# ViennaRNA/RNAcode

Measured on AMD Instinct MI355X. Metric: alignment-columns x samples scored /sec, higher is better.
Workload: dtype f32; 1 GPU; synthetic MAF 10000 blocks x 120 cols x 6 seqs, n=1000 (BASELINE configs[2]/[3]); exchange=none, fit_exp_mode=fused

## Files before the change

rnacode_amd/csrc/rc_null_kernel.h:

```cpp
#pragma once
#include <hip/hip_runtime.h>

#include <type_traits>
#include <utility>

#include "rc_device.h"
#include "rc_launch.h"

namespace rc {


template <bool SEM> __device__ __forceinline__ float ref_max(float x, float y) {
  if constexpr (SEM) return x > y ? x : y;
  else return fmaxf(x, y);
}
template <bool SEM> __device__ __forceinline__ float ref_max3(float x, float y, float z) { return ref_max<SEM>(ref_max<SEM>(x, y), z); }

template <bool SEM = false>
__device__ __forceinline__ void pair_step(int zc, float sig, float Delta, float Omega, float omega,
                                          float &s0, float &s1, float &s2) {
  if (zc == 0) {
    s0 = s0 + sig;
    s1 = s1 + omega;
    s2 = s2 + omega;
  } else if (zc == 1) {
    const float n0 = ref_max<SEM>(s0 + Delta, s2 + Omega);
    const float n1 = ref_max<SEM>(s0 + Omega, s1 + Delta);
    const float n2 = ref_max<SEM>(s1 + Omega, s2 + Delta);
    s0 = n0; s1 = n1; s2 = n2;
  } else {
    const float n0 = ref_max<SEM>(s0 + Delta, s1 + Omega);
    const float n1 = ref_max<SEM>(s1 + Delta, s2 + Omega);
    const float n2 = ref_max<SEM>(s2 + Delta, s0 + Omega);
    s0 = n0; s1 = n1; s2 = n2;
  }
}

struct ScanState {
  float cm;
  int ss, se;
};

template <typename Emit>
__device__ __forceinline__ void scan_step(ScanState &st, float v, int a, int j, bool last, float tieThr, Emit emit) {
  if (v > 0.0f || last) {
    if ((st.cm > 0.0f && st.se < a) || last) {
      if (st.se - st.ss >= 2) emit(st);
      st.cm = v; st.ss = a; st.se = j;
    } else if (v > st.cm || (fabsf(v - st.cm) < tieThr && (j - a) >= (st.se - st.ss))) {
      st.cm = v; st.ss = a; st.se = j;
    }
  }
}

__device__ __forceinline__ void native_scan_rows(const float *rows, int aLo, int aHi, int sites, int s, int f, float tieThr, ScanState &st, int &n,
                                                 DevHss *out, int hssCap, int lane) {
  for (int a = aLo; a < aHi; a++) {
    for (int j0 = a; j0 < sites; j0 += kWave) {
      const int j = j0 + lane;
      const float v = (j < sites) ? rows[static_cast<size_t>(a - aLo) * sites + j] : 0.0f;
      const bool last = (a == sites - 1) && (j == sites - 1);
      unsigned long long m = __ballot((j < sites) && (v > 0.0f || last));
      while (m) {
        const int t = __builtin_ctzll(m);
        m &= m - 1ull;
        const int jj = j0 + t;
        const float vt = __int_as_float(__builtin_amdgcn_readlane(__float_as_int(v), t));
        scan_step(st, vt, a, jj, (a == sites - 1) && (jj == sites - 1), tieThr, [&](const ScanState &e) {
          if (out && lane == 0 && n < hssCap) out[n] = DevHss{s, f, e.ss, e.se, e.cm};
          n++;
        });
      }
    }
  }
}

__device__ __forceinline__ uint32_t codon_flip(uint32_t c) { return ((c & 3u) << 4) | (c & 12u) | ((c >> 4) & 3u); }


template <int K> struct KReg { float s0, s1, s2; int lut; };
template <typename Seq> struct KRegs;
template <int... K> struct KRegs<std::integer_sequence<int, K...>> : KReg<K>... {
  template <int I> __device__ __forceinline__ KReg<I> &at() { return static_cast<KReg<I> &>(*this); }
};
template <int NK, typename F, int... K>
__device__ __forceinline__ void static_for_impl(F &&f, std::integer_sequence<int, K...>) {
  (f(std::integral_constant<int, K>{}), ...);
}
template <int NK, typename F> __device__ __forceinline__ void static_for(F &&f) {
  static_for_impl<NK>(static_cast<F &&>(f), std::make_integer_sequence<int, NK>{});
}

template <int NK, bool EXACT> __device__ __forceinline__ float div_by_nk(float x, float nkf) {
  if constexpr ((NK & (NK - 1)) == 0) {
    return x * (1.0f / static_cast<float>(NK));
  } else if constexpr (EXACT) {
    return x / nkf;
  } else {
    constexpr float y = 1.0f / static_cast<float>(NK);
    const float q0 = x * y;
    const float r = __builtin_fmaf(-static_cast<float>(NK), q0, x);
    return __builtin_fmaf(r, y, q0);
  }
}

struct SampleScan {
  float cm;
  float Q;
  uint32_t se;
  uint32_t len;
};
__device__ __forceinline__ void sample_scan_row_begin(SampleScan &st, float &best, uint32_t a) {
  const bool done = (st.cm > 0.0f) & (st.se < a);
  best = (done & (st.len >= 2u) & (st.cm > best)) ? st.cm : best;
  st.cm = done ? 0.0f : st.cm;
  st.len = done ? 0u : st.len;
  st.Q = static_cast<float>(2u * (st.len + a));
}
__device__ __forceinline__ void sample_scan_step(SampleScan &st, float v, float j2, float negTieThr) {
  const float d = v - st.cm;
  const bool upd = (v > st.cm) | ((v > 0.0f) & (d > negTieThr) & (st.Q <= j2));
  st.cm = upd ? v : st.cm;
  st.Q = upd ? j2 : st.Q;
}
__device__ __forceinline__ void sample_scan_row_end(SampleScan &st, uint32_t a) {
  const uint32_t q = static_cast<uint32_t>(st.Q);
  const bool inrow = (q & 1u) != 0u;
  const uint32_t j = q >> 1;
  st.se = inrow ? j : st.se;
  st.len = inrow ? j - a : st.len;
}
__device__ __forceinline__ void sample_scan_last(const SampleScan &st, float &best) {
  best = ((st.len >= 2u) & (st.cm > best)) ? st.cm : best;
}

struct DeepFetch {};
template <int OFF> struct StagedSite { uint32_t at; };
template <typename T> struct IsStagedSite : std::false_type {};
template <int OFF> struct IsStagedSite<StagedSite<OFF>> : std::true_type {};
template <int OFF> constexpr int staged_off(StagedSite<OFF>) { return OFF; }
__device__ __forceinline__ int site_index(int j) { return j; }
template <int OFF> __device__ __forceinline__ int site_index(StagedSite<OFF>) { return 0; }

template <int NK, bool LDSC, bool EXACT, bool DUAL, int MODE = 0>
__device__ __forceinline__ void null_body(const NullArgs &A, const uint8_t *__restrict__ blob,
                                          const DevBlock *__restrict__ dblocks, const int *__restrict__ classBlocks,
                                          const uint32_t *__restrict__ flags, const uint32_t *__restrict__ Ustream, const uint8_t *__restrict__ pairTab,
                                          uint32_t *__restrict__ scratch, float *__restrict__ maxima) {
  constexpr int N = NK + 1;
  constexpr int CPW = 5;
  constexpr int NCW = (NK + CPW - 1) / CPW;
  constexpr bool kTableLookups = !LDSC && !EXACT;
  constexpr int kTableWords = kTableLookups ? NK * kWave : 0;
  constexpr int LB = code_tail_bytes(NK);
  constexpr int PSW = code_pos_words(NK);
  using TailT = std::conditional_t<LB == 1, uint8_t, std::conditional_t<LB == 2, uint16_t, uint32_t>>;
  constexpr int ZW = (NK + 31) / 32;
  using Regs = KRegs<std::make_integer_sequence<int, NK>>;
  static_assert(!DUAL || (!EXACT && NK <= kDualRowsMaxNK), "two rows per pass: fast division, few sequences");
  static_assert(!(LDSC && EXACT), "the EXACT instantiation uses no LDS");
  constexpr bool ROWS = MODE == 1, SIM = MODE == 2;
#ifndef RC_DEEP_FETCH_MAX_NK
#define RC_DEEP_FETCH_MAX_NK 31
#endif
  constexpr bool kDeep = !LDSC && !EXACT && !DUAL && MODE == 0 && NK <= RC_DEEP_FETCH_MAX_NK;
  static_assert(MODE == 0 || (!LDSC && !EXACT && !DUAL), "rows split over workgroups: the one-row kernel that reads its codes from L2");
  extern __shared__ uint32_t lds_codes[];

  const int lane = threadIdx.x;
  unsigned int xcc;
  asm volatile("s_getreg_b32 %0, hwreg(HW_REG_XCC_ID)" : "=s"(xcc));
  const int home = static_cast<int>(xcc & 7u);
  const int rowParts = ROWS ? A.rowParts : 1;
  const int parts = SIM ? A.simParts : A.comboSplit ? 6 * rowParts : 1;
  const int nBlocks = A.nBlocksPtr ? *A.nBlocksPtr : A.nClassBlocks;
  const bool stealing = A.steal != nullptr && !A.comboSplit;
  constexpr int kStealHdr = 16;
  auto claim_part = [&](int slot) -> int {
    unsigned int v = 0;
    if (lane == 0) v = atomicAdd(A.steal + kStealHdr + slot, 1u);
    v = static_cast<unsigned int>(__builtin_amdgcn_readfirstlane(static_cast<int>(v)));
    return (v >= 1u && v <= 6u) ? static_cast<int>(v) - 1 : 6;
  };
  auto steal_word = [&](size_t at) -> unsigned int { return __hip_atomic_load(A.steal + at, __ATOMIC_RELAXED, __HIP_MEMORY_SCOPE_AGENT); };
  int helpCursor = 0;
  bool helping = false;
  for (int qi = 0;;) {
    int bi, grp, onlyCombo = -1, firstCombo = 0, rowPart = 0, itemIndex = 0;
    bool shared = false;
    int slot = static_cast<int>(blockIdx.x);
    if (!helping) {
      if (qi >= 8) {
        if (!stealing) break;
        helping = true;
        continue;
      }
      const int q = (home + qi) & 7;
      const int g0 = A.gLo + ((q - A.gLo) & 7);
      const int gq = g0 < A.gHi ? ((A.gHi - 1 - g0) >> 3) + 1 : 0;
      const int perBlock = gq * parts;
      const int nq = nBlocks * perBlock;
      int t = nq;
      if (nq > 0) {
        if (lane == 0) t = static_cast<int>(atomicAdd((SIM ? A.simCounter : A.workCounter) + q, 1u));
        t = __builtin_amdgcn_readfirstlane(t);
      }
      if (t >= nq) { qi++; continue; }
      bi = classBlocks[t / perBlock];
      if (A.skipMask && (flags[bi] & A.skipMask)) continue;
      const int sub = t % perBlock;
      grp = g0 + 8 * (sub / parts);
      onlyCombo = A.comboSplit ? (sub % parts) / rowParts : -1;
      if constexpr (MODE != 0) { rowPart = SIM ? sub % parts : (sub % parts) % rowParts; itemIndex = (t / perBlock) * (A.gHi - A.gLo) + (grp - A.gLo); }
      if constexpr (MODE != 0) slot = itemIndex;
      if (stealing && nq - t <= static_cast<int>(gridDim.x >> 3) + 16) {
        shared = true;
        if (lane == 0) atomicAdd(A.steal + 1, 1u);
      }
    } else {
      const size_t G = gridDim.x;
      const int np = __builtin_amdgcn_readfirstlane(static_cast<int>(steal_word(0)));
      int victim = -1;
      while (helpCursor < np) {
        const int i = helpCursor + lane;
        const unsigned int ent = i < np ? steal_word(kStealHdr + 3 * G + i) : 0u;
        const bool foreign = ent != 0u && (ent >> 24) != static_cast<unsigned int>(home);
        const unsigned int e = ent & 0xFFFFFFu;
        const unsigned int v = (e && !foreign) ? steal_word(kStealHdr + e - 1) : 0u;
        const unsigned long long open = __ballot(v >= 1u && v <= 6u);
        if (open) {
          int pick = static_cast<int>(blockIdx.x % static_cast<unsigned int>(__builtin_popcountll(open)));
          unsigned long long m = open;
          while (pick--) m &= m - 1ull;
          victim = __builtin_amdgcn_readlane(static_cast<int>(e), __builtin_ctzll(m)) - 1;
          break;
        }
        const unsigned long long notDone = ~__ballot(e != 0u && (v > 6u || foreign));
        const int adv = notDone ? __builtin_ctzll(notDone) : kWave;
        helpCursor += adv;
        if (adv < kWave) break;
      }
      if (victim < 0) {
        if (!A.stealWait) break;
        if (helpCursor >= np && steal_word(1) == 0u && static_cast<int>(steal_word(0)) == np) break;
        __builtin_amdgcn_s_sleep(127);
        continue;
      }
      firstCombo = claim_part(victim);
      if (firstCombo >= 6) continue;
      __atomic_thread_fence(__ATOMIC_ACQUIRE);
      shared = true;
      slot = victim;
      bi = __builtin_amdgcn_readfirstlane(static_cast<int>(steal_word(kStealHdr + G + 2 * victim)));
      grp = __builtin_amdgcn_readfirstlane(static_cast<int>(steal_word(kStealHdr + G + 2 * victim + 1)));
    }
    uint32_t *__restrict__ cod = scratch + static_cast<size_t>(slot) * A.scratchStride;
    const DevBlock *__restrict__ db = dblocks + bi;
    const bool nanSem = EXACT && (flags[bi] & kFlagNan) != 0u;
    const int cols = db->cols, L = db->L, nnodes = db->nnodes;
    const float Delta = db->Delta, Omega = db->Omega, omega = db->omega, nkf = db->nkf;
    const NodeRec *__restrict__ nodes = reinterpret_cast<const NodeRec *>(blob + db->off_nodes);
    const uint32_t *__restrict__ qtipw = reinterpret_cast<const uint32_t *>(blob + db->off_qtip);
    const uint32_t *__restrict__ refcolw = reinterpret_cast<const uint32_t *>(blob + db->off_refcol);
    const unsigned long long *__restrict__ zw = reinterpret_cast<const unsigned long long *>(blob + db->off_zw);
    const unsigned long long *__restrict__ zmask = reinterpret_cast<const unsigned long long *>(blob + db->off_zmask);
    const int zmWords = db->zm_words;
    const uint32_t *__restrict__ maskw = reinterpret_cast<const uint32_t *>(blob + db->off_mask);
    const float *__restrict__ lut = reinterpret_cast<const float *>(blob + db->off_lut);
    const int sidx = grp * kWave + lane;
    const int L1 = L + 1;

    if (!ROWS && !helping && (!kProfiling || !(A.debugSkip & 2))) {
      constexpr int SPI = 4;
      constexpr int NODEW = (2 * N - 1 + 15) / 16;
      const U4 *thrTab;
      const uint8_t *pairLut;
      int thrStride;
      if constexpr (EXACT) {
        thrTab = reinterpret_cast<const U4 *>(nodes);
        thrStride = sizeof(NodeRec) / sizeof(U4);
        pairLut = pairTab;
      } else {
        thrTab = reinterpret_cast<const U4 *>(lds_codes);
        thrStride = 4;
        pairLut = reinterpret_cast<const uint8_t *>(lds_codes + nnodes * 16);
        const uint32_t *src = reinterpret_cast<const uint32_t *>(nodes);
        for (int idx = lane; idx < nnodes * 16; idx += kWave) lds_codes[idx] = src[(idx >> 4) * (sizeof(NodeRec) / 4) + (idx & 15)];
        const uint32_t *psrc = reinterpret_cast<const uint32_t *>(pairTab);
#pragma unroll
        for (int x = 0; x < 64 * 64 / 4 / kWave; x++) lds_codes[nnodes * 16 + x * kWave + lane] = psrc[x * kWave + lane];
      }
      const uint32_t *__restrict__ nodew = reinterpret_cast<const uint32_t *>(nodes);
      uint32_t win[N];
#pragma unroll
      for (int r = 0; r < N; r++) win[r] = 0;
      unsigned int clamped = 0;
      auto get_state = [&](const uint32_t (&ns)[NODEW], int q) -> uint32_t {
        uint32_t word = ns[0];
#pragma unroll
        for (int x = 1; x < NODEW; x++) if ((q >> 4) == x) word = ns[x];
        return (word >> (2 * (q & 15))) & 3u;
      };
      int iLo = 1, iHi = L;
      if constexpr (SIM) { iLo = 1 + static_cast<int>(static_cast<long long>(L) * rowPart / parts); iHi = static_cast<int>(static_cast<long long>(L) * (rowPart + 1) / parts); }
      for (int i0 = (SIM && iLo > 3) ? iLo - 2 : 1; i0 <= iHi; i0 += SPI) {
        size_t ubase[SPI];
        uint32_t ns[SPI][NODEW];
#pragma unroll
        for (int t = 0; t < SPI; t++) {
          const int i = (i0 + t <= L) ? i0 + t : L;
          const uint32_t col = (refcolw[i >> 1] >> (16 * (i & 1))) & 0xFFFFu;
          ubase[t] = static_cast<size_t>(col) * A.Spad + sidx;
#pragma unroll
          for (int x = 0; x < NODEW; x++) ns[t][x] = 0;
        }
        const size_t qstride = static_cast<size_t>(cols) * A.Spad;
        auto node_step = [&](int q, const uint32_t (&u)[SPI]) {
          const uint32_t bp = nodew[q * 20 + 16];
          const int pq = static_cast<int>(nodew[q * 20 + 17] & 255u);
          auto evolve = [&](auto withBase) {
#pragma unroll
            for (int t = 0; t < SPI; t++) {
              const uint32_t ps = (q == 0) ? 0u : get_state(ns[t], pq);
              const U4 th = thrTab[q * thrStride + ps];
              uint32_t st = (u[t] > th.x) + (u[t] > th.y) + (u[t] > th.z);
              if constexpr (decltype(withBase)::value) st += (bp >> (2 * ps)) & 3u;
              if constexpr (SIM) clamped += (u[t] > th.w) & (i0 + t >= iLo) & (i0 + t <= iHi); else clamped += (u[t] > th.w);
              const uint32_t bits = st << (2 * (q & 15));
#pragma unroll
              for (int x = 0; x < NODEW; x++) if (NODEW == 1 || (q >> 4) == x) ns[t][x] |= bits;
            }
          };
          if (__builtin_expect(bp != 0u, 0)) evolve(std::true_type{}); else evolve(std::false_type{});
        };
        if constexpr (SIM) {
          constexpr int QB = 8;
          for (int q0 = 0; q0 < nnodes; q0 += QB) {
            uint32_t ub[QB][SPI];
#pragma unroll
            for (int x = 0; x < QB; x++) {
              const int q = q0 + x < nnodes ? q0 + x : nnodes - 1;
#pragma unroll
              for (int t = 0; t < SPI; t++) ub[x][t] = Ustream[ubase[t] + q * qstride];
            }
#pragma unroll
            for (int x = 0; x < QB; x++) if (q0 + x < nnodes) node_step(q0 + x, ub[x]);
          }
        } else {
          for (int q = 0; q < nnodes; q++) {
            uint32_t u[SPI];
#pragma unroll
            for (int t = 0; t < SPI; t++) u[t] = Ustream[ubase[t] + q * qstride];
            node_step(q, u);
          }
        }
#pragma unroll
        for (int t = 0; t < SPI; t++) {
          const int i = i0 + t;
          if (i <= L) {
#pragma unroll
            for (int r = 0; r < N; r++) win[r] = (win[r] << 2) | get_state(ns[t], static_cast<int>((qtipw[r >> 2] >> (8 * (r & 3))) & 255u));
            if (i >= 3 && (!SIM || (i >= iLo && i <= iHi))) {
              const int ip = L + 3 - i;
              const uint32_t aF = win[0] & 63u;
              const uint32_t aR = codon_flip(aF) ^ 63u;
#pragma unroll
              for (int w = 0; w < NCW; w++) {
                uint32_t wf = 0, wr = 0;
                const uint32_t mF = maskw[(0 * L1 + i) * NCW + w], mR = maskw[(1 * L1 + ip) * NCW + w];
#pragma unroll
                for (int c = 0; c < CPW; c++) {
                  const int k = w * CPW + c;
                  if (k < NK) {
                    const uint32_t bF = win[k + 1] & ((mF >> (6 * c)) & 63u);
                    const uint32_t bR = (codon_flip(win[k + 1]) ^ 63u) & ((mR >> (6 * c)) & 63u);
                    wf |= static_cast<uint32_t>(pairLut[aF * 64 + bF]) << (6 * c + 2);
                    wr |= static_cast<uint32_t>(pairLut[aR * 64 + bR]) << (6 * c + 2);
                  }
                }
                if (w < NCW - 1) {
                  cod[static_cast<size_t>(0 * L1 + i) * PSW + w * kWave + lane] = wf;
                  cod[static_cast<size_t>(1 * L1 + ip) * PSW + w * kWave + lane] = wr;
                } else {
                  reinterpret_cast<TailT *>(cod + static_cast<size_t>(0 * L1 + i) * PSW + (NCW - 1) * kWave)[lane] = static_cast<TailT>(wf);
                  reinterpret_cast<TailT *>(cod + static_cast<size_t>(1 * L1 + ip) * PSW + (NCW - 1) * kWave)[lane] = static_cast<TailT>(wr);
                }
              }
            }
          }
        }
      }
      if (clamped && sidx < A.sampleN && (SIM || onlyCombo <= 0)) atomicAdd(A.clampCount, static_cast<unsigned long long>(clamped));
    }
    if constexpr (SIM) continue;
    if (!helping && shared) {
      const size_t G = gridDim.x;
      if (lane == 0) {
        __hip_atomic_store(A.steal + kStealHdr + G + 2 * blockIdx.x, static_cast<unsigned int>(bi), __ATOMIC_RELAXED, __HIP_MEMORY_SCOPE_AGENT);
        __hip_atomic_store(A.steal + kStealHdr + G + 2 * blockIdx.x + 1, static_cast<unsigned int>(grp), __ATOMIC_RELAXED, __HIP_MEMORY_SCOPE_AGENT);
      }
      __builtin_amdgcn_fence(__ATOMIC_RELEASE, "agent");
      __builtin_amdgcn_s_waitcnt(0);
      if (lane == 0) {
        atomicExch(A.steal + kStealHdr + blockIdx.x, 1u);
        const unsigned int idx = atomicAdd(A.steal, 1u);
        __hip_atomic_store(A.steal + kStealHdr + 3 * G + idx, (blockIdx.x + 1u) | (static_cast<unsigned int>(home) << 24), __ATOMIC_RELAXED, __HIP_MEMORY_SCOPE_AGENT);
        atomicSub(A.steal + 1, 1u);
      }
      firstCombo = claim_part(slot);
    }

    float best = -1.0f;
    unsigned long long statCells = 0, statNoPos = 0, statPosLanes = 0, statPristine = 0, statEvent = 0, statTail = 0;
    float omega_v, Delta_v = 0.0f;
    asm volatile("v_mov_b32 %0, %1" : "=v"(omega_v) : "s"(omega));
    float rcpNk_v = 0.0f, negNk_v = 0.0f;
    if constexpr (!EXACT && (NK & (NK - 1)) != 0) {
      asm volatile("v_mov_b32 %0, %1" : "=v"(rcpNk_v) : "s"(1.0f / static_cast<float>(NK)));
      asm volatile("v_mov_b32 %0, %1" : "=v"(negNk_v) : "s"(-static_cast<float>(NK)));
    }
    if constexpr (EXACT) asm volatile("v_mov_b32 %0, %1" : "=v"(Delta_v) : "s"(Delta));
    if (!kProfiling || !(A.debugSkip & 1)) {
      Regs R;
      int curS = -1;
      for (int c = onlyCombo >= 0 ? onlyCombo : firstCombo; c < 6; c = onlyCombo >= 0 ? 6 : (shared ? claim_part(slot) : c + 1)) {
        const int s = c >= 3 ? 1 : 0, f = c - 3 * s;
        if (s != curS) {
          static_for<NK>([&](auto kc) {
            constexpr int k = decltype(kc)::value;
            R.template at<k>().lut = __float_as_int(lut[(s * NK + k) * kLutSize + lane]);
            if constexpr (kTableLookups) lds_codes[k * kWave + lane] = static_cast<uint32_t>(R.template at<k>().lut);
          });
          curS = s;
        }
        const int sites = (L - f) / 3;
        if (sites <= 0) continue;
        const uint32_t *__restrict__ sbase = cod + static_cast<size_t>(s * L1 + 3 + f) * PSW;
        constexpr int kSiteWords = 3 * PSW;
        auto word_at = [&](int j, int x) -> uint32_t {
          const uint32_t *p = sbase + static_cast<size_t>(j) * kSiteWords;
          if (x < NCW - 1) return p[x * kWave + lane];
          return static_cast<uint32_t>(reinterpret_cast<const TailT *>(p + (NCW - 1) * kWave)[lane]);
        };
        const unsigned long long *__restrict__ zbase = zw + static_cast<size_t>(s * L1 + 3 + f) * ZW;
        const unsigned long long *__restrict__ zany = zmask + static_cast<size_t>(s * 3 + f) * zmWords;
        int jc = sites;
        constexpr int kCacheSiteBytes = PSW * 4;
        if constexpr (LDSC) {
          for (int idx = 0; idx < sites * NCW; idx++) lds_codes[idx * kWave + lane] = word_at(idx / NCW, idx % NCW);
          __builtin_amdgcn_s_waitcnt(0);
        } else if constexpr (!EXACT) {
          jc = sites - (A.cacheSites < sites ? A.cacheSites : sites);
          for (int j = jc; j < sites; j++) {
            uint32_t *dst = lds_codes + kTableWords + (j - jc) * PSW;
#pragma unroll
            for (int x = 0; x < NCW - 1; x++) dst[x * kWave + lane] = word_at(j, x);
            reinterpret_cast<TailT *>(dst + (NCW - 1) * kWave)[lane] = static_cast<TailT>(word_at(j, NCW - 1));
          }
          __builtin_amdgcn_s_waitcnt(0);
        }
        const uint32_t ldsBase = static_cast<uint32_t>(reinterpret_cast<uintptr_t>(lds_codes + kTableWords));
        const uint32_t ldsLane = ldsBase + static_cast<uint32_t>(lane) * 4u;
        const uint32_t ldsTail = ldsBase + (NCW - 1) * kWave * 4u + static_cast<uint32_t>(lane) * LB;
        const uint32_t laneOff = static_cast<uint32_t>(lane) * 4u, laneTail = static_cast<uint32_t>(lane) * LB;
        [[maybe_unused]] const uint8_t *ldsBytesAll = reinterpret_cast<const uint8_t *>(lds_codes + kTableWords) - ldsBase;
        auto fetch_staged = [&](uint32_t (&w)[NCW], int j) {
          const uint32_t at = ldsLane + static_cast<uint32_t>(j) * (NCW * kWave * 4u);
#pragma unroll
          for (int x = 0; x < NCW; x++) {
#ifdef RC_PLAIN_FETCH
            w[x] = *reinterpret_cast<const uint32_t *>(ldsBytesAll + at + x * kWave * 4);
#else
            asm volatile("ds_read_b32 %0, %1 offset:%2" : "=v"(w[x]) : "v"(at), "n"(x * kWave * 4));
#endif
          }
        };
        auto fetch_staged_at = [&](uint32_t (&w)[NCW], auto site) {
          constexpr int off = staged_off(decltype(site){});
          static_assert(off + NCW * kWave * 4 <= 65536, "ds_read offset: 16 bits");
          const uint32_t at = site.at;
#pragma unroll
          for (int x = 0; x < NCW; x++) {
#ifdef RC_PLAIN_FETCH
            w[x] = *reinterpret_cast<const uint32_t *>(ldsBytesAll + at + off + x * kWave * 4);
#else
            asm volatile("ds_read_b32 %0, %1 offset:%2" : "=v"(w[x]) : "v"(at), "n"(off + x * kWave * 4));
#endif
          }
        };
        auto fetch_cached = [&](uint32_t (&w)[NCW], int j) {
          const uint32_t off = static_cast<uint32_t>(j - jc) * kCacheSiteBytes;
#ifdef RC_PLAIN_FETCH
          if constexpr (NCW > 1) {
#pragma unroll
            for (int x = 0; x < NCW - 1; x++) w[x] = *reinterpret_cast<const uint32_t *>(ldsBytesAll + ldsLane + off + x * kWave * 4);
          }
          w[NCW - 1] = static_cast<uint32_t>(*reinterpret_cast<const TailT *>(ldsBytesAll + ldsTail + off));
#else
          if constexpr (NCW > 1) {
            const uint32_t at = ldsLane + off;
#pragma unroll
            for (int x = 0; x < NCW - 1; x++) asm volatile("ds_read_b32 %0, %1 offset:%2" : "=v"(w[x]) : "v"(at), "n"(x * kWave * 4));
          }
          const uint32_t att = ldsTail + off;
          if constexpr (LB == 1) asm volatile("ds_read_u8 %0, %1" : "=v"(w[NCW - 1]) : "v"(att));
          else if constexpr (LB == 2) asm volatile("ds_read_u16 %0, %1" : "=v"(w[NCW - 1]) : "v"(att));
          else asm volatile("ds_read_b32 %0, %1" : "=v"(w[NCW - 1]) : "v"(att));
#endif
        };
        auto fetch_global = [&](uint32_t (&w)[NCW], const uint32_t *p) {
          const uint32_t lo = laneOff + 0u, lt = laneTail + 0u;
#ifdef RC_PLAIN_FETCH
          const uint8_t *pb = reinterpret_cast<const uint8_t *>(p);
#pragma unroll
          for (int x = 0; x < NCW - 1; x++) w[x] = *reinterpret_cast<const uint32_t *>(pb + lo + x * kWave * 4);
          w[NCW - 1] = static_cast<uint32_t>(*reinterpret_cast<const TailT *>(pb + lt + (NCW - 1) * kWave * 4));
          return;
#endif
#pragma unroll
          for (int x = 0; x < NCW - 1; x++) asm volatile("global_load_dword %0, %1, %2 offset:%3" : "=v"(w[x]) : "v"(lo), "s"(p), "n"(x * kWave * 4));
          if constexpr (LB == 1) asm volatile("global_load_ubyte %0, %1, %2 offset:%3" : "=v"(w[NCW - 1]) : "v"(lt), "s"(p), "n"((NCW - 1) * kWave * 4));
          else if constexpr (LB == 2) asm volatile("global_load_ushort %0, %1, %2 offset:%3" : "=v"(w[NCW - 1]) : "v"(lt), "s"(p), "n"((NCW - 1) * kWave * 4));
          else asm volatile("global_load_dword %0, %1, %2 offset:%3" : "=v"(w[NCW - 1]) : "v"(lt), "s"(p), "n"((NCW - 1) * kWave * 4));
        };
        auto load_words = [&](int j, uint32_t (&w)[NCW]) {
          if constexpr (LDSC) {
#pragma unroll
            for (int x = 0; x < NCW; x++) w[x] = lds_codes[(j * NCW + x) * kWave + lane];
          } else if constexpr (!EXACT) {
            if (j >= jc) {
              fetch_cached(w, j);
            } else {
              const uint32_t *p = sbase + static_cast<size_t>(j) * kSiteWords;
              asm volatile("s_nop 4" : "+s"(p));
              fetch_global(w, p);
            }
#pragma unroll
            for (int x = 0; x < NCW; x++) asm volatile("s_waitcnt vmcnt(0) lgkmcnt(0)" : "+v"(w[x]));
          } else {
#pragma unroll
            for (int x = 0; x < NCW; x++) w[x] = word_at(j, x);
          }
        };
        auto lookup = [&](uint32_t (&w)[NCW], float (&sig)[NK], auto jn, auto scalarLoadsNearby, auto kind) {
          if constexpr (LDSC) {
#pragma unroll
            for (int x = 0; x < NCW; x++) asm volatile("s_waitcnt lgkmcnt(0)" : "+v"(w[x]));
          }
          const uint32_t *pnext = sbase + static_cast<size_t>(site_index(jn)) * kSiteWords;
          if constexpr (!LDSC && !EXACT) asm volatile("" : "+s"(pnext));
          static_for<NK>([&](auto kc) {
            constexpr int k = decltype(kc)::value;
            constexpr int t = k % CPW;
            constexpr int kYounger = std::is_same_v<std::decay_t<decltype(kind)>, DeepFetch> ? NCW : 0;
            if constexpr (!LDSC && !EXACT && t == 0) asm volatile("s_waitcnt vmcnt(%1)" : "+v"(w[k / CPW]) : "n"(NCW - 1 - k / CPW + kYounger));
            uint32_t addr;
            if constexpr (t == 0) addr = w[k / CPW]; else addr = w[k / CPW] >> (6 * t);
            float got;
            if constexpr (kTableLookups) {
              uint32_t at;
              asm volatile("v_and_b32 %0, 0xfc, %1" : "=v"(at) : "v"(addr));
              asm volatile("ds_read_b32 %0, %1 offset:%2" : "=v"(got) : "v"(at), "n"(k * kWave * 4));
            } else {
              const int lutv = R.template at<k>().lut;
              asm volatile("ds_bpermute_b32 %0, %1, %2" : "=v"(got) : "v"(addr), "v"(lutv));
            }
            sig[k] = got;
          });
          auto wait_lookups = [&](auto leave) {
            constexpr int k0 = (NCW - 1) * CPW;
            constexpr int cnt = NK - k0;
            constexpr int left = (decltype(leave)::value > 0 && !decltype(scalarLoadsNearby)::value) ? decltype(leave)::value : 0;
            if constexpr (cnt == 1) asm volatile("s_waitcnt lgkmcnt(%1)" : "+v"(sig[k0]) : "n"(left));
            else if constexpr (cnt == 2) asm volatile("s_waitcnt lgkmcnt(%2)" : "+v"(sig[k0]), "+v"(sig[k0 + 1]) : "n"(left));
            else if constexpr (cnt == 3) asm volatile("s_waitcnt lgkmcnt(%3)" : "+v"(sig[k0]), "+v"(sig[k0 + 1]), "+v"(sig[k0 + 2]) : "n"(left));
            else if constexpr (cnt == 4)
              asm volatile("s_waitcnt lgkmcnt(%4)" : "+v"(sig[k0]), "+v"(sig[k0 + 1]), "+v"(sig[k0 + 2]), "+v"(sig[k0 + 3]) : "n"(left));
            else
              asm volatile("s_waitcnt lgkmcnt(%5)" : "+v"(sig[k0]), "+v"(sig[k0 + 1]), "+v"(sig[k0 + 2]), "+v"(sig[k0 + 3]), "+v"(sig[k0 + 4]) : "n"(left));
            static_for<NK>([&](auto kc) {
              constexpr int k = decltype(kc)::value;
              if constexpr (k < k0) {
                float b = sig[k];
                asm volatile("" : "+v"(b), "+v"(sig[k0]));
                sig[k] = b;
              }
            });
          };
          if constexpr (LDSC) {
            if constexpr (IsStagedSite<std::decay_t<decltype(jn)>>::value) fetch_staged_at(w, jn);
            else fetch_staged(w, jn);
            wait_lookups(std::integral_constant<int, NCW>{});
          } else if constexpr (!EXACT) {
            if constexpr (std::is_same_v<std::decay_t<decltype(kind)>, DeepFetch>) fetch_global(w, pnext);
            else if (jn >= jc) fetch_cached(w, jn);
            else fetch_global(w, pnext);
            wait_lookups(std::integral_constant<int, 0>{});
          } else {
            wait_lookups(std::integral_constant<int, 0>{});
          }
        };
        auto finish = [&](float sum) -> float {
          if constexpr (kProfiling) {
            const unsigned long long pos = __ballot(sum > 0.0f);
            statCells++; statNoPos += (pos == 0ull); statPosLanes += __builtin_popcountll(pos);
          }
          if constexpr (EXACT) {
            const float top = (sum > Delta_v) ? sum : Delta_v;
            return div_by_nk<NK, EXACT>(top, nkf);
          } else {
            if constexpr ((NK & (NK - 1)) == 0) return div_by_nk<NK, EXACT>(sum, nkf);
            else {
              const float q0 = sum * rcpNk_v;
              const float r = __builtin_fmaf(negNk_v, q0, sum);
              return __builtin_fmaf(r, rcpNk_v, q0);
            }
          }
        };
        auto fast_cell = [&](uint32_t (&w)[NCW], int jn, auto kind) -> float {
          float sig[NK];
          lookup(w, sig, jn, std::false_type{}, kind);
          float sum = 0.0f;
          static_for<NK>([&](auto kc) {
            constexpr int k = decltype(kc)::value;
            auto &r = R.template at<k>();
            r.s0 = r.s0 + sig[k];
            r.s1 = r.s1 + omega_v;
            r.s2 = r.s2 + omega_v;
            const float m = fmaxf(fmaxf(r.s0, r.s1), r.s2);
            sum = (k == 0) ? m : sum + m;
          });
          return finish(sum);
        };
        auto pristine_cell = [&](uint32_t (&w)[NCW], float &wv, int jn, auto kind) -> float {
          float sig[NK];
          lookup(w, sig, jn, std::false_type{}, kind);
          wv = wv + omega_v;
          float sum = 0.0f;
          static_for<NK>([&](auto kc) {
            constexpr int k = decltype(kc)::value;
            auto &r = R.template at<k>();
            r.s0 = r.s0 + sig[k];
            const float m = fmaxf(r.s0, wv);
            sum = (k == 0) ? m : sum + m;
          });
          return finish(sum);
        };
        auto tail_cell = [&](uint32_t (&w)[NCW], int jn, auto kind) -> float {
          float sig[NK];
          lookup(w, sig, jn, std::false_type{}, kind);
          float sum = 0.0f;
          static_for<NK>([&](auto kc) {
            constexpr int k = decltype(kc)::value;
            auto &r = R.template at<k>();
            r.s0 = r.s0 + sig[k];
            r.s1 = r.s1 + omega_v;
            const float m = fmaxf(r.s0, r.s1);
            sum = (k == 0) ? m : sum + m;
          });
          return finish(sum);
        };
        auto event_cell = [&](uint32_t (&w)[NCW], int j, int jn, auto kind, auto sem) -> float {
          constexpr bool SEM = decltype(sem)::value;
          float sig[NK];
          lookup(w, sig, jn, std::true_type{}, kind);
          unsigned long long z[ZW];
#pragma unroll
          for (int x = 0; x < ZW; x++) z[x] = zbase[static_cast<size_t>(3 * j) * ZW + x];
          float sum = 0.0f;
          static_for<NK>([&](auto kc) {
            constexpr int k = decltype(kc)::value;
            auto &r = R.template at<k>();
            pair_step<SEM>(static_cast<int>((z[k >> 5] >> (2 * (k & 31))) & 3ull), sig[k], Delta, Omega, omega, r.s0, r.s1, r.s2);
            const float m = ref_max3<SEM>(r.s0, r.s1, r.s2);
            sum = (k == 0) ? m : sum + m;
          });
          return finish(sum);
        };
// ... 508 lines not shown
```

Measured before the change: 28.20 billion alignment-columns*samples/s.

## Hand-tune null-sample evolution loop with buffer loads, inline-asm compares, reversed window

Rewrites the per-node state evolution in the null-sample kernel. Draw loads now go through buffer resource descriptors with 32-bit offsets. The four-site threshold compares become hand-written inline assembly that carry-adds the compare results and builds a wave-wide clamp mask, so the clamp counting only runs when some lane exceeds the clamp threshold. Parent indices are packed into a 64-bit register when the tree fits one word, and node records are prefetched otherwise. A reversed codon window is kept alongside the forward one so codon_flip is no longer computed per pair. This cuts address arithmetic, scalar loads and ALU work in the hot loop, at the cost of inline-asm fragility, assumptions about SPI==4 and the descriptor range, and extra registers.

Result: no change. 28.48 billion alignment-columns*samples/s, median of 6 (+1.0%).

```diff
diff --git a/rnacode_amd/csrc/rc_null_kernel.h b/rnacode_amd/csrc/rc_null_kernel.h
--- a/rnacode_amd/csrc/rc_null_kernel.h
+++ b/rnacode_amd/csrc/rc_null_kernel.h
@@ -291,9 +291,9 @@
         for (int x = 0; x < 64 * 64 / 4 / kWave; x++) lds_codes[nnodes * 16 + x * kWave + lane] = psrc[x * kWave + lane];
       }
       const uint32_t *__restrict__ nodew = reinterpret_cast<const uint32_t *>(nodes);
-      uint32_t win[N];
-#pragma unroll
-      for (int r = 0; r < N; r++) win[r] = 0;
+      uint32_t win[N], winR[N];
+#pragma unroll
+      for (int r = 0; r < N; r++) win[r] = winR[r] = 0;
       unsigned int clamped = 0;
       auto get_state = [&](const uint32_t (&ns)[NODEW], int q) -> uint32_t {
         uint32_t word = ns[0];
@@ -303,35 +303,80 @@
       };
       int iLo = 1, iHi = L;
       if constexpr (SIM) { iLo = 1 + static_cast<int>(static_cast<long long>(L) * rowPart / parts); iHi = static_cast<int>(static_cast<long long>(L) * (rowPart + 1) / parts); }
+      unsigned long long parPack = 0;
+      uint32_t bpAny = 0;
+      if constexpr (NODEW == 1 && !SIM) {
+        for (int q = 0; q < nnodes; q++) {
+          parPack |= static_cast<unsigned long long>(nodew[q * 20 + 17] & 15u) << (4 * q);
+          bpAny |= nodew[q * 20 + 16];
+        }
+      }
       for (int i0 = (SIM && iLo > 3) ? iLo - 2 : 1; i0 <= iHi; i0 += SPI) {
         size_t ubase[SPI];
+        uint32_t ucol[SPI];
         uint32_t ns[SPI][NODEW];
 #pragma unroll
         for (int t = 0; t < SPI; t++) {
           const int i = (i0 + t <= L) ? i0 + t : L;
           const uint32_t col = (refcolw[i >> 1] >> (16 * (i & 1))) & 0xFFFFu;
           ubase[t] = static_cast<size_t>(col) * A.Spad + sidx;
+          ucol[t] = col * static_cast<uint32_t>(A.Spad) * 4u;
 #pragma unroll
           for (int x = 0; x < NODEW; x++) ns[t][x] = 0;
         }
         const size_t qstride = static_cast<size_t>(cols) * A.Spad;
-        auto node_step = [&](int q, const uint32_t (&u)[SPI]) {
-          const uint32_t bp = nodew[q * 20 + 16];
-          const int pq = static_cast<int>(nodew[q * 20 + 17] & 255u);
-          auto evolve = [&](auto withBase) {
+        const bool drawsByDescriptor = qstride * sizeof(uint32_t) <= 0xFFFFFFFFull;
+        const int drawBytes = drawsByDescriptor ? static_cast<int>(static_cast<uint32_t>(qstride * sizeof(uint32_t))) : 0;
+        auto draws_of = [&](int q, uint32_t (&u)[SPI]) {
+          const uint32_t *uq = Ustream + q * qstride;
+          const auto rsrc = __builtin_amdgcn_make_buffer_rsrc(const_cast<uint32_t *>(uq), 0, drawBytes, 0x00020000);
+#pragma unroll
+          for (int t = 0; t < SPI; t++) u[t] = __builtin_amdgcn_raw_buffer_load_b32(rsrc, sidx * 4, static_cast<int>(ucol[t]), 0);
+          if (__builtin_expect(!drawsByDescriptor, 0)) {
+#pragma unroll
+            for (int t = 0; t < SPI; t++) u[t] = uq[ubase[t]];
+          }
+        };
+        auto node_step = [&](int q, uint32_t bp, int pq, const uint32_t (&u)[SPI]) {
+          uint32_t st[SPI];
+          U4 th[SPI];
+#pragma unroll
+          for (int t = 0; t < SPI; t++) {
+            th[t] = thrTab[q * thrStride + ((q == 0) ? 0u : get_state(ns[t], pq))];
+            st[t] = th[t].x;
+          }
+          static_assert(SPI == 4, "the compares are written out for four sites");
+          unsigned long long any, mask;
+          asm("v_cmp_gt_u32_e64 vcc, %6, %0\n\tv_cmp_gt_u32_e64 %4, %7, %1\n\tv_cmp_gt_u32_e64 %5, %8, %2\n\tv_cndmask_b32_e64 %0, 0, 1, vcc\n\t"
+              "v_cmp_gt_u32_e64 vcc, %9, %3\n\tv_cndmask_b32_e64 %1, 0, 1, %4\n\tv_cndmask_b32_e64 %2, 0, 1, %5\n\tv_cndmask_b32_e64 %3, 0, 1, vcc\n\t"
+              "v_cmp_gt_u32_e64 %4, %6, %10\n\tv_cmp_gt_u32_e64 %5, %7, %13\n\tv_cmp_gt_u32_e64 vcc, %8, %16\n\tv_addc_co_u32_e64 %0, %4, 0, %0, %4\n\t"
+              "v_cmp_gt_u32_e64 %4, %9, %19\n\tv_addc_co_u32_e64 %1, %5, 0, %1, %5\n\tv_addc_co_u32_e64 %2, vcc, 0, %2, vcc\n\tv_addc_co_u32_e64 %3, %4, 0, %3, %4\n\t"
+              "v_cmp_gt_u32_e64 %5, %6, %11\n\tv_cmp_gt_u32_e64 vcc, %7, %14\n\tv_cmp_gt_u32_e64 %4, %8, %17\n\tv_addc_co_u32_e64 %0, %5, 0, %0, %5\n\t"
+              "v_cmp_gt_u32_e64 %5, %9, %20\n\tv_addc_co_u32_e64 %1, vcc, 0, %1, vcc\n\tv_addc_co_u32_e64 %2, %4, 0, %2, %4\n\tv_addc_co_u32_e64 %3, %5, 0, %3, %5\n\t"
+              "v_cmp_gt_u32_e64 vcc, %6, %12\n\tv_cmp_gt_u32_e64 %4, %7, %15\n\tv_cmp_gt_u32_e64 %5, %8, %18\n\ts_or_b64 %4, %4, vcc\n\t"
+              "v_cmp_gt_u32_e64 vcc, %9, %21\n\ts_or_b64 %4, %4, %5\n\ts_or_b64 %4, %4, vcc"
+              : "+v"(st[0]), "+v"(st[1]), "+v"(st[2]), "+v"(st[3]), "=&s"(any), "=&s"(mask)
+              : "v"(u[0]), "v"(u[1]), "v"(u[2]), "v"(u[3]), "v"(th[0].y), "v"(th[0].z), "v"(th[0].w), "v"(th[1].y), "v"(th[1].z), "v"(th[1].w),
+                "v"(th[2].y), "v"(th[2].z), "v"(th[2].w), "v"(th[3].y), "v"(th[3].z), "v"(th[3].w)
+              : "vcc");
+          if (__builtin_expect(any != 0ull, 0)) {
 #pragma unroll
             for (int t = 0; t < SPI; t++) {
-              const uint32_t ps = (q == 0) ? 0u : get_state(ns[t], pq);
-              const U4 th = thrTab[q * thrStride + ps];
-              uint32_t st = (u[t] > th.x) + (u[t] > th.y) + (u[t] > th.z);
-              if constexpr (decltype(withBase)::value) st += (bp >> (2 * ps)) & 3u;
-              if constexpr (SIM) clamped += (u[t] > th.w) & (i0 + t >= iLo) & (i0 + t <= iHi); else clamped += (u[t] > th.w);
-              const uint32_t bits = st << (2 * (q & 15));
-#pragma unroll
-              for (int x = 0; x < NODEW; x++) if (NODEW == 1 || (q >> 4) == x) ns[t][x] |= bits;
-            }
-          };
-          if (__builtin_expect(bp != 0u, 0)) evolve(std::true_type{}); else evolve(std::false_type{});
+              if constexpr (SIM) clamped += (u[t] > th[t].w) & (i0 + t >= iLo) & (i0 + t <= iHi); else clamped += (u[t] > th[t].w);
+            }
+          }
+          if (__builtin_expect(bp != 0u, 0)) {
+            int pqAgain = pq;
+            asm volatile("" : "+s"(pqAgain));
+#pragma unroll
+            for (int t = 0; t < SPI; t++) st[t] += (bp >> (2 * ((q == 0) ? 0u : get_state(ns[t], pqAgain)))) & 3u;
+          }
+#pragma unroll
+          for (int t = 0; t < SPI; t++) {
+            const uint32_t bits = st[t] << (2 * (q & 15));
+#pragma unroll
+            for (int x = 0; x < NODEW; x++) if (NODEW == 1 || (q >> 4) == x) ns[t][x] |= bits;
+          }
         };
         if constexpr (SIM) {
           constexpr int QB = 8;
@@ -340,18 +385,35 @@
 #pragma unroll
             for (int x = 0; x < QB; x++) {
               const int q = q0 + x < nnodes ? q0 + x : nnodes - 1;
-#pragma unroll
-              for (int t = 0; t < SPI; t++) ub[x][t] = Ustream[ubase[t] + q * qstride];
-            }
-#pragma unroll
-            for (int x = 0; x < QB; x++) if (q0 + x < nnodes) node_step(q0 + x, ub[x]);
+              draws_of(q, ub[x]);
+            }
+#pragma unroll
+            for (int x = 0; x < QB; x++)
+              if (q0 + x < nnodes) node_step(q0 + x, nodew[(q0 + x) * 20 + 16], static_cast<int>(nodew[(q0 + x) * 20 + 17] & 255u), ub[x]);
           }
         } else {
-          for (int q = 0; q < nnodes; q++) {
-            uint32_t u[SPI];
-#pragma unroll
-            for (int t = 0; t < SPI; t++) u[t] = Ustream[ubase[t] + q * qstride];
-            node_step(q, u);
+          if constexpr (NODEW == 1) {
+            for (int q = 0; q < nnodes; q++) {
+              uint32_t u[SPI];
+              draws_of(q, u);
+              uint32_t bp = 0;
+              if (__builtin_expect(bpAny != 0u, 0)) bp = nodew[q * 20 + 16];
+              node_step(q, bp, static_cast<int>((parPack >> (4 * q)) & 15ull), u);
+            }
+          } else {
+            const uint32_t *nrec = nodew + 16;
+            uint32_t bpNext = nrec[0], pqNext = nrec[1];
+            for (int q = 0; q < nnodes; q++) {
+              uint32_t u[SPI];
+              draws_of(q, u);
+              asm volatile("" : "+s"(bpNext), "+s"(pqNext));
+              const uint32_t bp = bpNext;
+              const int pq = static_cast<int>(pqNext & 255u);
+              nrec += (q + 1 < nnodes) ? 20 : 0;
+              bpNext = nrec[0];
+              pqNext = nrec[1];
+              node_step(q, bp, pq, u);
+            }
           }
         }
 #pragma unroll
@@ -359,11 +421,15 @@
           const int i = i0 + t;
           if (i <= L) {
 #pragma unroll
-            for (int r = 0; r < N; r++) win[r] = (win[r] << 2) | get_state(ns[t], static_cast<int>((qtipw[r >> 2] >> (8 * (r & 3))) & 255u));
+            for (int r = 0; r < N; r++) {
+              const uint32_t tip = get_state(ns[t], static_cast<int>((qtipw[r >> 2] >> (8 * (r & 3))) & 255u));
+              win[r] = (win[r] << 2) | tip;
+              winR[r] = (winR[r] >> 2) | (tip << 4);
+            }
             if (i >= 3 && (!SIM || (i >= iLo && i <= iHi))) {
               const int ip = L + 3 - i;
               const uint32_t aF = win[0] & 63u;
-              const uint32_t aR = codon_flip(aF) ^ 63u;
+              const uint32_t aR = winR[0] ^ 63u;
 #pragma unroll
               for (int w = 0; w < NCW; w++) {
                 uint32_t wf = 0, wr = 0;
@@ -373,7 +439,7 @@
                   const int k = w * CPW + c;
                   if (k < NK) {
                     const uint32_t bF = win[k + 1] & ((mF >> (6 * c)) & 63u);
-                    const uint32_t bR = (codon_flip(win[k + 1]) ^ 63u) & ((mR >> (6 * c)) & 63u);
+                    const uint32_t bR = (winR[k + 1] ^ 63u) & ((mR >> (6 * c)) & 63u);
                     wf |= static_cast<uint32_t>(pairLut[aF * 64 + bF]) << (6 * c + 2);
                     wr |= static_cast<uint32_t>(pairLut[aR * 64 + bR]) << (6 * c + 2);
                   }
```
